# snap-research/F8Net

Measured on AMD Instinct MI355X. Metric: images/sec at bs=128 (ResNet-50 INT8), higher is better.
Workload: dtype int8 x int8 -> int32 (exact integer)

## Files before the change

### f8net_amd/csrc/f8_internal.h

```cpp
#pragma once
#include <hip/hip_runtime.h>
#include <stdint.h>
#include <stddef.h>

namespace f8 {

struct Options {
    int split = 2;
    int fuse_blocks = 1;
    int fuse_stages = -1;
    int fuse_dual = 1;
    int fuse_ds = 1;
    int fuse_opener = 1;
    int fuse_fc = 1;
    int fuse_stem = 1;
    int fuse_input = 1;
    int wstat = 1;
    int wstat_min_tiles = 2;
    int wstat_fast = 1;
    int s2wreg = 1;
    int wreg = 1;
    int fuse_bchain = 2;
    int fuse_bchain7 = 0;
    int fuse_chain = 1;
    int fuse_chain7 = 1;
    int fuse_pool = 1;
    int fuse_tail = 1;
    int chain_timeout_ms = 10000;
    int chain_stack = 1;
    int fuse_p12 = 1;
    int fuse_head2 = 1;
    int fuse_ir = 1;
    int fuse_irchain = 0;
    int fuse_dws = 0;
    int fuse_head_dws = 0;
    int fuse_dws7 = 0;
    int patch3x3 = 1;
    int dual_wide = 2048;
    int deep_nk = 7;
    int bk128 = 0;
    int dw_dot4 = 1;
    int dwk_dot4 = 1;
    int dw_mma = 1;
    int stem_rows = 1;
    int stem_grid_div = 0;
    int stem_wpc = 3;
    int opener_stg = 1;
    int chunk56 = -1, chunk28 = -1, chunk14 = -1;
    int chunk_budget_mb = 96;
    int chunk_ds = 1, chunk_opener = 0;
    int whole_batch_launches = 0;
    int pipeline_depth = 2;
    int shared_streams = 1;
    int arena_copies = 0;
    int split_streams = 1;
    int graph = 0;
    int stagger = -1, stagger_pipelined = 2;
    int check_device = 1;
    int requant_float = 0;
    int tap_tiled = 1;
    int check_input_range = 1;
};
void options_from_env(Options* o);
int* option_slot(Options* o, const char* key);

struct QuantOut {
    int8_t* ptr;
    int32_t n;
    int32_t lo, hi;
    uint32_t bias_xor;
// ... 274 lines not shown
inline bool dyn_lds_opted_in(unsigned long long* done, int* dev_out) {
    int dev = 0;
    if (hipGetDevice(&dev) != hipSuccess || dev < 0 || dev >= 64) { *dev_out = -1; return false; }
    *dev_out = dev;
    return ((*done >> dev) & 1ull) != 0;
}

struct ConvTile { int bm, bn, bk; };


bool pick_conv_tile(int M, int coutP, int ck, bool has_res, bool bk128, ConvTile* t);
int  conv_grid(const ConvTile& t, int M, int coutP);

int conv_inst(const ConvArgs& a, const ConvTile& t, bool res, bool dual, int deep_nk);
int conv_kernel_name(char* buf, size_t cap, const ConvArgs& a, const ConvTile& t, int inst);
hipError_t launch_conv(const ConvArgs& a, const ConvTile& t, int inst, hipStream_t s);
hipError_t launch_fused_bottleneck(const FusedArgs& a, hipStream_t s);
int fused_bottleneck_kernel_name(char* buf, size_t cap, const FusedArgs& a);
bool fused_bottleneck_supported(int C, int MID, int H, int W, int imgs_per_launch, int stage_mask, int* R);
bool fused_ds_supported(int C, int MID, int COUT, int H, int W, int* R);
bool fused_opener_supported(int C, int MID, int COUT, int H, int W, int* R);
int fused_opener_inst(const FusedArgs& a, bool stg);
int fused_opener_kernel_name(char* buf, size_t cap, const FusedArgs& a, int inst);
hipError_t launch_fused_opener(const FusedArgs& a, int inst, hipStream_t s);
bool chain_supported(int C, int MID, int H, int W, int cin0);
bool chain_tail_supported(int C, int MID, int H, int W, int cin0);
int chain_max_blocks(int C, int MID, int H, int W, int cin0, bool tail);
void chain_shape(int C, int MID, int H, int W, int cin0, bool tail, int* R, int* wg_per_cu);
bool chain_stackable(int C, int MID, int H, int W, int cin0, bool tail);
hipError_t launch_chain(const ChainArgs& a, int fast, int C, int MID, int H, int W, int cin0, hipStream_t s);
int chain_kernel_name(char* buf, size_t cap, int C, int MID, int H, int W, int cin0, bool tail, int fast);
bool cchain_supported(int C, int MID, int H, int W, int cin0, bool tail);
size_t cchain_xchg_bytes();
int cchain_clusters(int N, int slots);
int cchain_kernel_name(char* buf, size_t cap, int fast);
int chain_fast(const ChainArgs& a, unsigned shortcut_blocks, bool q8);
hipError_t launch_cchain(const ChainArgs& a, int fast, hipStream_t s);
bool bcchain_supported(int C, int H, int W, bool opener);
size_t bcchain_xchg_bytes();
int bcchain_inst(const BCChainArgs& a, bool q8);
int bcchain_kernel_name(char* buf, size_t cap, int inst);
hipError_t launch_bcchain(const BCChainArgs& a, int inst, hipStream_t s);
bool bchain_supported(int C, int H, int W);
bool bchain_ds_supported(int C, int H, int W);
int bchain_tiles_per_img(int C, int H, int W);
hipError_t launch_bchain(const BChainArgs& a, int fast, int C, int H, int W, hipStream_t s);
int bchain_fast(const BChainArgs& a, bool ds, bool q8);
// ... 79 lines not shown
```

### f8net_amd/csrc/f8_net.cpp

```cpp
#include "../../include/f8net.h"
#include "f8_internal.h"

#include <algorithm>
#include <cstdarg>
#include <cstdio>
#include <cstdlib>
#include <cstring>
#include <new>
#include <variant>
#include <string>
#include <mutex>
#include <vector>

using namespace f8;

namespace {

thread_local std::string g_err;

int fail(int code, const char* fmt, ...) {
    char buf[512];
    va_list ap;
    va_start(ap, fmt);
    vsnprintf(buf, sizeof buf, fmt, ap);
// ... 251 lines not shown
    {"fuse_tail", "F8_FUSE_TAIL", &Options::fuse_tail, 0, 1, true},
    {"fuse_chain7", "F8_FUSE_CHAIN7", &Options::fuse_chain7, 0, 1, true},
    {"fuse_pool", "F8_FUSE_POOL", &Options::fuse_pool, 0, 1, true},
    {"fuse_bchain", "F8_FUSE_BCHAIN", &Options::fuse_bchain, 0, 2, true},
    {"fuse_bchain7", "F8_FUSE_BCHAIN7", &Options::fuse_bchain7, 0, 2, true},
    {"chain_timeout_ms", "F8_CHAIN_TIMEOUT_MS", &Options::chain_timeout_ms, 0, 1 << 20, false},
    {"chain_stack", "F8_CHAIN_STACK", &Options::chain_stack, 0, 1, true},
    {"wreg", "F8_WREG", &Options::wreg, 0, 1, true},
    {"s2wreg", "F8_S2WREG", &Options::s2wreg, 0, 1, true},
    {"wstat", "F8_WSTAT", &Options::wstat, 0, 1, true},
    {"wstat_min_tiles", "F8_WSTAT_MIN_TILES", &Options::wstat_min_tiles, 0, 1 << 20, true},
    {"wstat_fast", "F8_WSTAT_FAST", &Options::wstat_fast, 0, 1, true},
    {"patch3x3", "F8_PATCH3X3", &Options::patch3x3, 0, 1, true},
    {"dual_wide", "F8_DUAL_WIDE", &Options::dual_wide, 0, 1 << 30, true},
    {"deep_nk", "F8_DEEP_NK", &Options::deep_nk, 1, 1 << 20, true},
    {"bk128", "F8_BK128", &Options::bk128, 0, 1, true},
    {"dw_dot4", "F8_DW_DOT4", &Options::dw_dot4, 0, 1, true},
    {"dw_mma", "F8_DW_MMA", &Options::dw_mma, 0, 1, true},
    {"dwk_dot4", "F8_DWK_DOT4", &Options::dwk_dot4, 0, 1, true},
    {"stem_wpc", "F8_STEM_WPC", &Options::stem_wpc, 1, 8, false},
    {"stem_rows", "F8_STEM_ROWS", &Options::stem_rows, 0, 1, true},
    {"stem_grid_div", "F8_STEM_GRID_DIV", &Options::stem_grid_div, 0, 32, false},
    {"opener_stg", "F8_OPENER_STG", &Options::opener_stg, 0, 1, true},
    {"chunk56", "F8_CHUNK", &Options::chunk56, -1, 1 << 20, false},
    {"chunk28", "F8_CHUNK28", &Options::chunk28, -1, 1 << 20, false},
    {"chunk14", "F8_CHUNK14", &Options::chunk14, -1, 1 << 20, false},
    {"chunk_budget_mb", "F8_CHUNK_BUDGET_MB", &Options::chunk_budget_mb, 1, 1 << 20, false},
    {"chunk_ds", "F8_CHUNK_DS", &Options::chunk_ds, 0, 1, false},
    {"chunk_opener", "F8_CHUNK_OPENER", &Options::chunk_opener, 0, 1, false},
    {"split_streams", "F8_SPLIT_STREAMS", &Options::split_streams, 0, 1, false},
    {"graph", "F8_GRAPH", &Options::graph, 0, 1, false},
    {"stagger", "F8_STAGGER", &Options::stagger, -1, 1 << 20, false},
    {"stagger_pipelined", "F8_STAGGER_PIPELINED", &Options::stagger_pipelined, 0, 1 << 20, false},
    {"check_device", "F8_CHECK_DEVICE", &Options::check_device, 0, 1, false},
    {"check_input_range", "F8_CHECK_INPUT_RANGE", &Options::check_input_range, 0, 1, false},
    {"requant_float", "F8_REQUANT_FLOAT", &Options::requant_float, 0, 1, true},
    {"pipeline_depth", "F8_PIPELINE_DEPTH", &Options::pipeline_depth, 2, 4, false},
    {"arena_copies", "F8_ARENA_COPIES", &Options::arena_copies, 0, 4, true},
    {"shared_streams", "F8_SHARED_STREAMS", &Options::shared_streams, 0, 1, true},
    {"whole_batch_launches", "F8_WHOLE_BATCH_LAUNCHES", &Options::whole_batch_launches, 0, 1, true},
    {"tap_tiled", "F8_TAP_TILED", &Options::tap_tiled, 0, 1, true},
};
static const OptKey* find_opt(const char* key) {
    if (!key) return nullptr;
    for (const auto& k : kOptKeys) if (!strcmp(k.key, key)) return &k;
    return nullptr;
// ... 2495 lines not shown
            a.x = (const int8_t*)fp(sF); a.x_bytes = (uint32_t)(sF.bytes_per_img * N); a.N = N;
            if (st.kind == S_STEMPOOL) a.wpc = net->opt.stem_wpc;
            a.grid_div = net->opt.stem_grid_div;
            if (st.raw_input && !(net->in_u8 && net->in_u8_nhwc)) {
                const size_t img = (size_t)sT.C * sT.H * sT.W;
                a.rC = sT.C; a.rH = sT.H; a.rW = sT.W; a.xor8 = sF.sgn ? 0u : 0x80808080u;
                if (net->in_u8) { a.raw_kind = 2; a.xu8 = net->in_u8 + (size_t)n0 * img; memcpy(a.lut, net->in_lut, sizeof a.lut); }
                else if (net->in_f32) { a.raw_kind = 1; a.xf = net->in_f32 + (size_t)n0 * img; a.scale = net->in_scale; a.qlo = net->in_lo; a.qhi = net->in_hi; }
                else {
                    a.raw_kind = 0; a.xi = input + (size_t)n0 * img;
                    if (net->opt.check_input_range) { a.err = net->d_err; a.chk_lo = sF.sgn ? -127 : 0; a.chk_hi = sF.sgn ? 127 : 255; }
                }
            }
            fill_out(&a.out32, a.q);
            e = launch_stem_pool(a, st.inst, s);
            break;
        }
        case S_FUSED: case S_P12: {
            const Form& xF = T[st.src_t].forms[st.src_f];
            FusedArgs a = std::get<FusedArgs>(st.args);
            a.x8 = (const int8_t*)fp(xF); a.x_bytes = (uint32_t)(xF.bytes_per_img * N); a.N = N;
            if (st.res_t >= 0) a.xr = (const int32_t*)fp(T[st.res_t].forms[st.res_f]);
            fill_out(&a.out32, a.q);
            e = st.variant == V_OPENER ? launch_fused_opener(a, st.inst, s) : st.variant == V_P12 ? launch_fused_p12(a, s) : launch_fused_bottleneck(a, s);
            break;
        }
        case S_CHAIN: {
            ChainArgs a = std::get<ChainArgs>(st.args);
            const Form& xF = T[st.src_t].forms[st.src_f];
            if (xF.kind == FORM_I8) a.x8in = (const int8_t*)fp(xF); else a.xr = (const int32_t*)fp(xF);
            if (a.tail) a.m2in = (const int8_t*)fp(T[st.src2_t].forms[st.src2_f]);
            a.N = N;
            if ((a.NG = chain_launch_groups(net, st, N, &a.stack)) < 1) return F8_ERR_STATE;
            fill_out(&a.out32, a.q);
            if (const int rc = chain_scratch(a.cs)) return rc;
            e = launch_chain(a, st.inst, st.C, st.MID, st.H, st.W, st.cin0, s);
            break;
        }
        case S_BCHAIN: if (st.cluster) {
            BCChainArgs a = std::get<BCChainArgs>(st.args);
            const Tensor& xs = T[st.src_t];
            if (st.res_t >= 0) { a.m0in = (const int8_t*)fp(xs.forms[st.src_f]); a.x8sc = (const int8_t*)fp(T[st.res_t].forms[st.res_f]); }
            else a.xr = (const int32_t*)fp(xs.forms[st.src_f]);
            a.N = N;
            { int32_t one = 1; if ((a.NG = chain_launch_groups(net, st, N, &one)) < 1) return F8_ERR_STATE; }
            fill_out(&a.out32, a.q);
            if (const int rc = chain_scratch(a.cs)) return rc;
// ... 518 lines not shown
```

### f8net_amd/csrc/f8_opener.hip

```cpp
#include "f8_device.h"
#include <cstdlib>
#include <cstdio>

namespace f8 {

template <int C, int MID, int W, int R, int COUT>
struct OpenerCfg {
    static constexpr int WO = W / 2;
    static constexpr int PR = 2 * R + 1;
    static constexpr int NE = WO + 1, NO = WO;
    static constexpr int PW = NE + NO;
    static constexpr int P1_PX = PR * W, NP1 = (P1_PX + 31) / 32;
    static constexpr int OUT_PX = R * WO, NPO = (OUT_PX + 31) / 32;
    static constexpr int PATCH_BYTES = (PR * PW * MID + 255) / 256 * 256;
    static constexpr int X1_BYTES = NP1 * 32 * 64, W0_BYTES = MID * 64, STAGE1 = X1_BYTES + W0_BYTES;
    static constexpr int MID2_BYTES = NPO * 32 * MID, XS_BYTES = NPO * 32 * C;
    static constexpr int W2B = MID * 64, NS2 = 5;
    static constexpr int REG_B = MID2_BYTES + XS_BYTES + NS2 * W2B;
    static constexpr int REG_A = 2 * STAGE1 > REG_B ? 2 * STAGE1 : REG_B;
    static constexpr int BIAS_INTS = 2 * MID + 2 * COUT;
    static constexpr int LDS_BYTES = PATCH_BYTES + REG_A + BIAS_INTS * 4;
    static constexpr int STAGE3 = 64 * MID + 64 * C;
    static constexpr int STG_BYTES = NPO * 32 * 128;
};

template <int C, int MID, int W, int R, int COUT, bool STG, bool P12 = false, int FQ = 0>
__global__ void __launch_bounds__(512) __attribute__((amdgpu_waves_per_eu(2, 2)))
fused_opener_kernel(const FusedArgs a) {
    using Cfg = OpenerCfg<C, MID, W, R, COUT>;
    constexpr int WO = Cfg::WO, PR = Cfg::PR, NE = Cfg::NE, PW = Cfg::PW;
    constexpr int P1_PX = Cfg::P1_PX, NP1 = Cfg::NP1, OUT_PX = Cfg::OUT_PX, NPO = Cfg::NPO;
    constexpr int CM = MID / 32, CMW = CM / 2, NP1W = (NP1 + 3) / 4;
    constexpr int NK1 = C / 64, NK2 = 9 * (MID / 64), NC3 = COUT / 64, KK3 = MID / 32, KKS = C / 32, CH = MID / 64;
    constexpr int X1_BYTES = Cfg::X1_BYTES, STAGE1 = Cfg::STAGE1, W2B = Cfg::W2B, NS2 = Cfg::NS2, STAGE3 = Cfg::STAGE3;
    static_assert(NPO == 4 && CM % 2 == 0 && NP1 % 4 == 0, "4 pixel-tile groups x 2 channel-tile groups");
    static_assert(MID % 64 == 0 && C % 64 == 0 && COUT % 128 == 0, "K steps of 64 bytes, chunk pairs");
    static_assert(Cfg::LDS_BYTES <= 160 * 1024, "LDS");
    static_assert(2 * STAGE3 <= Cfg::PATCH_BYTES && STAGE3 <= NS2 * W2B, "P3 ring: two stages over the patch, one over the W2 ring");
    static_assert(!STG || (Cfg::PATCH_BYTES - 2 * STAGE3 >= Cfg::STG_BYTES && NS2 * W2B - STAGE3 >= Cfg::STG_BYTES), "staging buffers");
    constexpr int XL1 = X1_BYTES / 16 / 512;
    constexpr int WL0 = (MID * 4 + 511) / 512;
    constexpr int WL4 = 64 * MID / 16 / 512, WLS = 64 * C / 16 / 512, XSL = NPO * 32 * C / 16 / 512;
    static_assert(X1_BYTES % 8192 == 0 && (MID * 4) % 512 == 0 && WL4 >= 1 && WLS >= 1, "every wave issues every DMA instruction (compile-time wait counts)");
    constexpr int L1 = XL1 + WL0, L3 = WL4 + WLS;

    if constexpr (FQ == 1) set_fp_round_nearest_even();
    extern __shared__ __attribute__((aligned(16))) char lds[];
    char* const patch = lds;
    char* const regA = lds + Cfg::PATCH_BYTES;
    char* const mid2 = regA;
    char* const xs = regA + Cfg::MID2_BYTES;
    char* const w2ring = xs + Cfg::XS_BYTES;
    int* const bias_lds = (int*)(regA + Cfg::REG_A);
    auto p3slot = [&](int s) -> char* { return s < 2 ? patch + s * STAGE3 : w2ring; };
    auto stgbuf = [&](int b) -> char* { return b == 0 ? patch + 2 * STAGE3 : w2ring + STAGE3; };

    using S64 = Swz<64>;
    using SM = Swz<MID>;
    using SC = Swz<C>;

    const int tid = threadIdx.x;
    const int lane = tid & 63;
    const int wave = __builtin_amdgcn_readfirstlane(tid >> 6) & 7;
    const int wa = wave >> 1, wb = wave & 1;
    const int l31 = lane & 31, lh = lane >> 5;

    int t;
    {
        const int nwg = gridDim.x, bid = blockIdx.x, xcd = bid & 7, qq = nwg >> 3, rr = nwg & 7;
        t = (xcd < rr ? xcd * (qq + 1) : rr * (qq + 1) + (xcd - rr) * qq) + (bid >> 3);
    }
    const int HO = a.H >> 1;
    const int n = t / a.tiles_per_img, ti = t - n * a.tiles_per_img;
    const int p0 = ti * R;
    const int gp1 = (n * a.H + 2 * p0 - 1) * W;
    const int m_tile = (n * HO + p0) * WO;

    const __amdgpu_buffer_rsrc_t rx = __builtin_amdgcn_make_buffer_rsrc((void*)a.x8, 0, a.x_bytes, 0x00020000);
    const __amdgpu_buffer_rsrc_t rw0 = __builtin_amdgcn_make_buffer_rsrc((void*)a.w0, 0, a.w0_bytes, 0x00020000);
    const __amdgpu_buffer_rsrc_t rw2 = __builtin_amdgcn_make_buffer_rsrc((void*)a.w2, 0, a.w2_bytes, 0x00020000);
    const __amdgpu_buffer_rsrc_t rw4 = __builtin_amdgcn_make_buffer_rsrc((void*)a.w4, 0, a.w4_bytes, 0x00020000);
    const __amdgpu_buffer_rsrc_t rwsc = __builtin_amdgcn_make_buffer_rsrc((void*)a.wsc, 0, a.wsc_bytes, 0x00020000);

#ifdef F8_TRACE
    unsigned long long tt[8]; tt[0] = __builtin_readcyclecounter();
#define F8_OT(i) tt[i] = __builtin_readcyclecounter()
#else
#define F8_OT(i)
#endif

    for (int i = tid; i < (P12 ? 2 * MID : Cfg::BIAS_INTS); i += 512) {
        int v;
        if (i < MID) v = a.b0[i];
        else if (i < 2 * MID) v = a.b2[i - MID];
        else if (i < 2 * MID + COUT) v = a.b4[i - 2 * MID];
        else v = a.bsc[i - 2 * MID - COUT];
        bias_lds[i] = v;
    }
    {
        const unsigned z = a.xor1;
        const v4i zv = {(int)z, (int)z, (int)z, (int)z};
        if (tid < PR * (MID / 16)) *(v4i*)(patch + (tid / (MID / 16)) * PW * MID + (tid % (MID / 16)) * 16) = zv;
        if (p0 == 0)
            for (int o = tid * 16; o < PW * MID; o += 512 * 16) *(v4i*)(patch + o) = zv;
    }

    unsigned xb1[XL1];
#pragma unroll
    for (int i = 0; i < XL1; ++i) {
        const int idx = tid + i * 512;
        const int row = idx >> 2, chunk = (idx & 3) ^ S64::f(row);
        const int pr = row / W;
        const bool ok = row < P1_PX && (2 * p0 - 1 + pr) >= 0;
        xb1[i] = ok ? (unsigned)((gp1 + row) * C + chunk * 16) : kOOB;
// ... 59 lines not shown
        char* base = p3slot(slot);
#pragma unroll
        for (int j = 0; j < WL4; ++j) {
            const unsigned woff = w4b[j] + (unsigned)(c * 64 * MID);
            __builtin_amdgcn_raw_ptr_buffer_load_lds(rw4, (__attribute__((address_space(3))) void*)(base + j * 8192 + wave * 1024), 16, woff, 0, 0, 0);
        }
#pragma unroll
        for (int j = 0; j < WLS; ++j) {
            const unsigned woff = wsb[j] + (unsigned)(c * 64 * C);
            __builtin_amdgcn_raw_ptr_buffer_load_lds(rwsc, (__attribute__((address_space(3))) void*)(base + 64 * MID + j * 8192 + wave * 1024), 16, woff, 0, 0, 0);
        }
    };

    unsigned cof[2];
#pragma unroll
    for (int kk = 0; kk < 2; ++kk) cof[kk] = (unsigned)(((kk * 2 + lh) ^ S64::f(l31)) << 4);

    {
        v16i acc[NP1W][CMW];
#pragma unroll
        for (int i = 0; i < CMW; ++i)
#pragma unroll
            for (int g = 0; g < 4; ++g) {
                v4i bv = {0, 0, 0, 0};
                if constexpr (FQ != 0) bv = *(const v4i*)(a.b0 + (wb * CMW + i) * 32 + 8 * g + 4 * lh);
#pragma unroll
                for (int j = 0; j < NP1W; ++j)
#pragma unroll
                    for (int e = 0; e < 4; ++e) acc[j][i][4 * g + e] = bv[e];
            }
        issue_p1(0, 0);
        static_for<NK1>([&](auto kc) {
            constexpr int KS = decltype(kc)::value;
            wait_vmcnt<0>();
            asm volatile("s_waitcnt lgkmcnt(0)" ::: "memory");
            __builtin_amdgcn_s_barrier();
            if constexpr (KS + 1 < NK1) issue_p1(KS + 1, (KS + 1) & 1);
            const char* base = regA + (KS & 1) * STAGE1;
#pragma unroll
            for (int kk = 0; kk < 2; ++kk) {
                v4i wf[CMW], xf[NP1W];
#pragma unroll
                for (int i = 0; i < CMW; ++i) wf[i] = *(const v4i*)(base + X1_BYTES + ((wb * CMW + i) * 32 + l31) * 64 + cof[kk]);
#pragma unroll
                for (int j = 0; j < NP1W; ++j) xf[j] = *(const v4i*)(base + ((wa + 4 * j) * 32 + l31) * 64 + cof[kk]);
#pragma unroll
                for (int j = 0; j < NP1W; ++j)
#pragma unroll
                    for (int i = 0; i < CMW; ++i) acc[j][i] = __builtin_amdgcn_mfma_i32_32x32x32_i8(wf[i], xf[j], acc[j][i], 0, 0, 0);
            }
        });
        asm volatile("s_waitcnt lgkmcnt(0)" ::: "memory");
        __builtin_amdgcn_s_barrier();
        F8_OT(1);
        if constexpr (!P12) issue_xs();
#pragma unroll
        for (int k = 0; k < NS2 - 1; ++k) issue_w2(k, k);

        const int floor0 = a.relu_a ? 0 : INT32_MIN;
        const float sc1 = FQ == 1 ? requant_u8_scale(a.n1) : 0.0f;
        (void)floor0; (void)sc1;
#pragma unroll
        for (int j = 0; j < NP1W; ++j) {
            const int pix = (wa + 4 * j) * 32 + l31;
            const int pr = pix / W, pc = pix - pr * W + 1;
            const bool ok = pix < P1_PX && (2 * p0 - 1 + pr) >= 0;
            const int ent = pr * PW + ((pc & 1) ? NE + (pc >> 1) : (pc >> 1));
#pragma unroll
            for (int i = 0; i < CMW; ++i) {
                const int ct = wb * CMW + i;
                unsigned d[4];
#pragma unroll
                for (int g = 0; g < 4; ++g) {
                    if constexpr (FQ != 0) {
                        d[g] = requant_u8x4_sel<FQ == 2 ? 2 : 1>(acc[j][i][4 * g], acc[j][i][4 * g + 1], acc[j][i][4 * g + 2], acc[j][i][4 * g + 3], a.n1, sc1) ^ 0x80808080u;
                    } else {
                        const v4i bv = *(const v4i*)(bias_lds + ct * 32 + 8 * g + 4 * lh);
                        int y[4];
#pragma unroll
                        for (int e = 0; e < 4; ++e) y[e] = requant1(max((int)((unsigned)acc[j][i][4 * g + e] + (unsigned)bv[e]), floor0), a.n1, a.lo1, a.hi1);
                        d[g] = pack4(y[0], y[1], y[2], y[3]) ^ a.xor1;
                    }
                }
                auto s0 = __builtin_amdgcn_permlane32_swap(d[0], d[2], false, false);
                auto s1 = __builtin_amdgcn_permlane32_swap(d[1], d[3], false, false);
                if (ok) {
                    v4i o = {(int)s0[0], (int)s0[1], (int)s1[0], (int)s1[1]};
                    *(v4i*)(patch + SM::off(ent, ct * 2 + lh)) = o;
                }
            }
        }
    }
    F8_OT(2);

    const int opix = wa * 32 + l31;
    const bool opix_ok = opix < OUT_PX;
    const int m = m_tile + opix;

    {
        v16i acc[CMW];
        const int oc = opix_ok ? opix : OUT_PX - 1;
        const int orow = oc / WO, ocol = oc - orow * WO;
        const int pe[3] = {2 * orow * PW + ocol, 2 * orow * PW + NE + ocol, 2 * orow * PW + ocol + 1};
#pragma unroll
        for (int i = 0; i < CMW; ++i)
// ... 7 lines not shown
            constexpr int J = decltype(jc)::value;
            constexpr int BEFORE = J == 0 ? NS2 - 1 : ((J - 1 + NS2 < NK2) ? J - 1 + NS2 : NK2);
            constexpr int AFTER = (J + NS2 < NK2) ? J + NS2 : NK2;
            wait_vmcnt<(BEFORE - 1 - J) * WL0>();
            asm volatile("s_waitcnt lgkmcnt(0)" ::: "memory");
            __builtin_amdgcn_s_barrier();
            static_for<AFTER - BEFORE>([&](auto ic) { constexpr int S = BEFORE + decltype(ic)::value; issue_w2(S, S % NS2); });
            constexpr int TAP = J / CH, TC = J % CH, TR = TAP / 3, TS = TAP % 3;
            const char* base = w2ring + (J % NS2) * W2B;
            const int ent = pe[TS] + TR * PW;
#pragma unroll
            for (int kk = 0; kk < 2; ++kk) {
                const v4i xf = *(const v4i*)(patch + SM::off(ent, TC * 4 + kk * 2 + lh));
#pragma unroll
                for (int i = 0; i < CMW; ++i) {
                    const v4i wf = *(const v4i*)(base + ((wb * CMW + i) * 32 + l31) * 64 + cof[kk]);
                    acc[i] = __builtin_amdgcn_mfma_i32_32x32x32_i8(wf, xf, acc[i], 0, 0, 0);
                }
            }
        });
        F8_OT(3);
        asm volatile("s_waitcnt lgkmcnt(0)" ::: "memory");
        __builtin_amdgcn_s_barrier();
        if constexpr (!P12) {
            issue_p3(0, 0);
            asm volatile("" ::: "memory");
            issue_p3(1, 1);
            asm volatile("" ::: "memory");
        }

        const int floor0 = a.relu_b ? 0 : INT32_MIN;
        const float sc2 = FQ == 1 ? requant_u8_scale(a.n2) : 0.0f;
        (void)floor0; (void)sc2;
#pragma unroll
        for (int i = 0; i < CMW; ++i) {
            const int ct = wb * CMW + i;
            unsigned d[4];
#pragma unroll
            for (int g = 0; g < 4; ++g) {
                if constexpr (FQ != 0) {
                    d[g] = requant_u8x4_sel<FQ == 2 ? 2 : 1>(acc[i][4 * g], acc[i][4 * g + 1], acc[i][4 * g + 2], acc[i][4 * g + 3], a.n2, sc2) ^ 0x80808080u;
                } else {
                    int y[4];
#pragma unroll
                    for (int e = 0; e < 4; ++e) y[e] = requant1(max(acc[i][4 * g + e], floor0), a.n2, a.lo2, a.hi2);
                    d[g] = pack4(y[0], y[1], y[2], y[3]) ^ a.xor2;
                }
            }
            auto s0 = __builtin_amdgcn_permlane32_swap(d[0], d[2], false, false);
            auto s1 = __builtin_amdgcn_permlane32_swap(d[1], d[3], false, false);
            v4i o = {(int)s0[0], (int)s0[1], (int)s1[0], (int)s1[1]};
            if constexpr (P12) { if (opix_ok) *(v4i*)(a.q[0].ptr + (size_t)m * MID + ct * 32 + lh * 16) = o; }
            else *(v4i*)(mid2 + SM::off(opix, ct * 2 + lh)) = o;
        }
    }
    F8_OT(4);

    if constexpr (!P12) {
        const int floor1 = a.relu1 ? 0 : -2147483647 ;
        const bool stage0 = STG && a.q[0].ptr != nullptr;
        const int n_direct = (a.out32 ? 4 : 0) + ((!STG && a.q[0].ptr) ? 1 : 0) + (a.q[1].ptr ? 1 : 0);
        auto stores_of = [&](int x) { return x < 0 ? 0 : n_direct + ((stage0 && x >= 2 && !(x & 1)) ? 2 : 0); };
        auto flush_pair = [&](int c0) {
            const char* buf = stgbuf((c0 >> 1) & 1);
#pragma unroll
            for (int rr = 0; rr < 2; ++rr) {
                const int tq = tid + rr * 512;
                const int row = tq >> 3, c16 = tq & 7;
                const bool live = row < OUT_PX;
                const int rw = live ? row : OUT_PX - 1;
                if (live || lane == 0) {
                    const v4i v = *(const v4i*)(buf + rw * 128 + ((c16 ^ (rw & 7)) << 4));
                    *(v4i*)(a.q[0].ptr + (size_t)(m_tile + rw) * COUT + c0 * 64 + c16 * 16) = v;
                }
            }
        };
        v4i xf[KK3], xsf[KKS];
        static_for<NC3>([&](auto cc) {
            constexpr int c = decltype(cc)::value;
            wait_vmcnt_dyn(stores_of(c - 2) + (c + 1 < NC3 ? L3 : 0) + stores_of(c - 1));
            asm volatile("s_waitcnt lgkmcnt(0)" ::: "memory");
// ... 58 lines not shown
                    *(v4i*)(stgbuf((c >> 1) & 1) + opix * 128 + ((c16 ^ (opix & 7)) << 4)) = o;
                } else if (opix_ok) {
                    *(v4i*)(a.q[k].ptr + (size_t)m * COUT + cot + 16 * lh) = o;
                }
            }
        });
        if (stage0) {
            asm volatile("s_waitcnt lgkmcnt(0)" ::: "memory");
            __builtin_amdgcn_s_barrier();
            flush_pair(NC3 - 2);
        }
    }
#ifdef F8_TRACE
    if (a.trace && tid == 0) {
        asm volatile("s_waitcnt vmcnt(0)" ::: "memory");
        tt[5] = __builtin_readcyclecounter();
        unsigned long long* tp = (unsigned long long*)a.trace + (size_t)blockIdx.x * 8;
        for (int i = 0; i < 6; ++i) tp[i] = tt[i];
    }
#endif
}

template <int C, int MID, int W, int R, int COUT, bool STG, bool P12 = false, int FQ = 0>
static hipError_t launch_opener_t(const FusedArgs& a, hipStream_t s) {
    using Cfg = OpenerCfg<C, MID, W, R, COUT>;
    static unsigned long long attr_done = 0; int attr_dev = -1;
    if (!dyn_lds_opted_in(&attr_done, &attr_dev)) {
        hipError_t e = hipFuncSetAttribute((const void*)fused_opener_kernel<C, MID, W, R, COUT, STG, P12, FQ>, hipFuncAttributeMaxDynamicSharedMemorySize, Cfg::LDS_BYTES);
        if (e != hipSuccess) return e;
        if (attr_dev >= 0) attr_done |= 1ull << attr_dev;
    }
    const int grid = a.N * a.tiles_per_img;
#ifdef F8_TRACE
    static unsigned long long* tbuf = nullptr; static int count = 0;
    static const int want = [] { const char* e = getenv("F8_TRACE_OPENER"); return e ? atoi(e) : -1; }();
    FusedArgs b = a;
    const bool tracing = (count++ == want);
    if (tracing) { if (!tbuf) (void)hipMalloc((void**)&tbuf, (size_t)1 << 22); (void)hipMemsetAsync(tbuf, 0, (size_t)grid * 64, s); b.trace = tbuf; }
    hipLaunchKernelGGL((fused_opener_kernel<C, MID, W, R, COUT, STG, P12, FQ>), dim3(grid), dim3(512), Cfg::LDS_BYTES, s, b);
    if (tracing) {
        (void)hipStreamSynchronize(s);
        unsigned long long* h = new unsigned long long[(size_t)grid * 8];
        (void)hipMemcpy(h, tbuf, (size_t)grid * 64, hipMemcpyDeviceToHost);
        double ph[5] = {0, 0, 0, 0, 0}; int n = 0;
        for (int i = 0; i < grid; ++i) { unsigned long long* p = h + (size_t)i * 8; if (!p[5]) continue; ++n; for (int k = 0; k < 5; ++k) ph[k] += (double)(p[k + 1] - p[k]); }
        fprintf(stderr, "[trace opener<%d,%d,%d,%d,%d>] grid %d: avg cycles per WG: P1 loop %.0f | P1 epi %.0f | P2 loop %.0f | P2 epi %.0f | P3 %.0f\n", C, MID, W, R, COUT, grid,
                ph[0] / n, ph[1] / n, ph[2] / n, ph[3] / n, ph[4] / n);
        delete[] h;
    }
    return hipGetLastError();
#else
    hipLaunchKernelGGL((fused_opener_kernel<C, MID, W, R, COUT, STG, P12, FQ>), dim3(grid), dim3(512), Cfg::LDS_BYTES, s, a);
    return hipGetLastError();
#endif
}

int fused_opener_inst(const FusedArgs& a, bool stg) {
    if (!a.p12only) return stg ? 1 : 0;
    const bool fqf = a.relu_a && a.relu_b && a.n1 > 0 && a.n2 > 0 && a.n1 <= 30 && a.n2 <= 30 && a.lo1 == 0 && a.lo2 == 0 && a.hi1 == 255 && a.hi2 == 255 &&
                     a.xor1 == 0x80808080u && a.xor2 == 0x80808080u;
#ifndef F8_OPENER_FQ
#define F8_OPENER_FQ 1
#endif
    return (!fqf || !F8_OPENER_FQ) ? 0 : ((a.rq_int || !a.acc_ok || a.n1 > kRequantU8MaxShift || a.n2 > kRequantU8MaxShift) ? 2 : 1);
}

int fused_opener_kernel_name(char* buf, size_t cap, const FusedArgs& a, int inst) {
    return snprintf(buf, cap, "f8::fused_opener_kernel<%d, %d, %d, %d, %d, %s, %s, %d>", a.C, a.MID, a.W, a.R, a.COUT, !a.p12only && inst ? "true" : "false",
                    a.p12only ? "true" : "false", a.p12only ? inst : 0);
}

hipError_t launch_fused_opener(const FusedArgs& a, int inst, hipStream_t s) {
    if (a.C == 256 && a.MID == 128 && a.COUT == 512 && a.W == 56 && a.R == 4) {
        if (a.p12only) {
            if (!(a.q[0].ptr && !a.q[1].ptr && !a.out32)) return hipErrorInvalidValue;
            const int fq = inst;
            return fq == 1 ? launch_opener_t<256, 128, 56, 4, 512, false, true, 1>(a, s) : fq == 2 ? launch_opener_t<256, 128, 56, 4, 512, false, true, 2>(a, s)
                                                                                               : launch_opener_t<256, 128, 56, 4, 512, false, true, 0>(a, s);
        }
        return inst ? launch_opener_t<256, 128, 56, 4, 512, true>(a, s) : launch_opener_t<256, 128, 56, 4, 512, false>(a, s);
    }
    return hipErrorInvalidValue;
}

bool fused_opener_supported(int C, int MID, int COUT, int H, int W, int* R) {
    if (C == 256 && MID == 128 && COUT == 512 && W == 56 && H % 8 == 0) { *R = 4; return true; }
    return false;
}

}
```

Baseline: 161,200.

## Make P12 opener kernel persistent with cross-tile prefetch of next tile's P1 stages

Splits the P12-only opener path into a dedicated persistent device routine. Each workgroup loops over a contiguous range of tiles (XCD-aware assignment), and the grid is capped at the CU count, optionally lower via a new F8_OPENER_WGS option. The first P1 stages of the next tile are issued during and after the current tile's P2, and biases are staged in LDS once per workgroup, so launch and pipeline fill costs are hidden. The trade-off is fewer workgroups, a tighter LDS ring layout with more complex vmcnt accounting, and possible load imbalance across tiles.

```diff
diff --git a/f8net_amd/csrc/f8_internal.h b/f8net_amd/csrc/f8_internal.h
--- a/f8net_amd/csrc/f8_internal.h
+++ b/f8net_amd/csrc/f8_internal.h
@@ -46,6 +46,7 @@
     int stem_grid_div = 0;
     int stem_wpc = 3;
     int opener_stg = 1;
+    int opener_wgs = 0;
     int chunk56 = -1, chunk28 = -1, chunk14 = -1;
     int chunk_budget_mb = 96;
     int chunk_ds = 1, chunk_opener = 0;
@@ -366,7 +367,7 @@
 bool fused_opener_supported(int C, int MID, int COUT, int H, int W, int* R);
 int fused_opener_inst(const FusedArgs& a, bool stg);
 int fused_opener_kernel_name(char* buf, size_t cap, const FusedArgs& a, int inst);
-hipError_t launch_fused_opener(const FusedArgs& a, int inst, hipStream_t s);
+hipError_t launch_fused_opener(const FusedArgs& a, int inst, int num_cu, int opener_wgs, hipStream_t s);
 bool chain_supported(int C, int MID, int H, int W, int cin0);
 bool chain_tail_supported(int C, int MID, int H, int W, int cin0);
 int chain_max_blocks(int C, int MID, int H, int W, int cin0, bool tail);
diff --git a/f8net_amd/csrc/f8_net.cpp b/f8net_amd/csrc/f8_net.cpp
--- a/f8net_amd/csrc/f8_net.cpp
+++ b/f8net_amd/csrc/f8_net.cpp
@@ -297,6 +297,7 @@
     {"stem_rows", "F8_STEM_ROWS", &Options::stem_rows, 0, 1, true},
     {"stem_grid_div", "F8_STEM_GRID_DIV", &Options::stem_grid_div, 0, 32, false},
     {"opener_stg", "F8_OPENER_STG", &Options::opener_stg, 0, 1, true},
+    {"opener_wgs", "F8_OPENER_WGS", &Options::opener_wgs, 0, 256, false},
     {"chunk56", "F8_CHUNK", &Options::chunk56, -1, 1 << 20, false},
     {"chunk28", "F8_CHUNK28", &Options::chunk28, -1, 1 << 20, false},
     {"chunk14", "F8_CHUNK14", &Options::chunk14, -1, 1 << 20, false},
@@ -2838,7 +2839,7 @@
             a.x8 = (const int8_t*)fp(xF); a.x_bytes = (uint32_t)(xF.bytes_per_img * N); a.N = N;
             if (st.res_t >= 0) a.xr = (const int32_t*)fp(T[st.res_t].forms[st.res_f]);
             fill_out(&a.out32, a.q);
-            e = st.variant == V_OPENER ? launch_fused_opener(a, st.inst, s) : st.variant == V_P12 ? launch_fused_p12(a, s) : launch_fused_bottleneck(a, s);
+            e = st.variant == V_OPENER ? launch_fused_opener(a, st.inst, net->num_cu, net->opt.opener_wgs, s) : st.variant == V_P12 ? launch_fused_p12(a, s) : launch_fused_bottleneck(a, s);
             break;
         }
         case S_CHAIN: {
diff --git a/f8net_amd/csrc/f8_opener.hip b/f8net_amd/csrc/f8_opener.hip
--- a/f8net_amd/csrc/f8_opener.hip
+++ b/f8net_amd/csrc/f8_opener.hip
@@ -24,6 +24,298 @@
     static constexpr int STG_BYTES = NPO * 32 * 128;
 };
 
+template <int C, int MID, int W, int R, int COUT, int FQ>
+__device__ __forceinline__ void opener_p12_tiles(const FusedArgs& a, char* const lds) {
+    using Cfg = OpenerCfg<C, MID, W, R, COUT>;
+    constexpr int WO = Cfg::WO, PR = Cfg::PR, NE = Cfg::NE, PW = Cfg::PW;
+    constexpr int P1_PX = Cfg::P1_PX, NP1 = Cfg::NP1, OUT_PX = Cfg::OUT_PX;
+    constexpr int CM = MID / 32, CMW = CM / 2, NP1W = (NP1 + 3) / 4;
+    constexpr int NK1 = C / 64, NK2 = 9 * (MID / 64), CH = MID / 64;
+    constexpr int X1_BYTES = Cfg::X1_BYTES, STAGE1 = Cfg::STAGE1, W2B = Cfg::W2B, NS2 = Cfg::NS2;
+    constexpr int XL1 = X1_BYTES / 16 / 512, WL0 = (MID * 4 + 511) / 512, L1 = XL1 + WL0;
+    constexpr int NST = CMW;
+    static_assert(STAGE1 <= Cfg::PATCH_BYTES && 2 * STAGE1 <= Cfg::REG_A, "P1 ring: slots 0 and 1 in REG_A, slot 2 over the patch");
+    static_assert(STAGE1 <= Cfg::MID2_BYTES + Cfg::XS_BYTES, "slot 0 (the next tile's stage 0, in flight during P2) lies below the W2 ring");
+    static_assert(NK1 >= 3 && NK2 > NS2 && OUT_PX > 3 * 32, "three stages up front; a prefetch step inside P2; no wave without a live output pixel");
+    static_assert(P1_PX > (XL1 - 1) * 128 && W <= 128, "dead gather rows: only in the last DMA instruction; image row -1: only in the first");
+
+    if constexpr (FQ == 1) set_fp_round_nearest_even();
+    char* const patch = lds;
+    char* const regA = lds + Cfg::PATCH_BYTES;
+    char* const w2ring = regA + Cfg::MID2_BYTES + Cfg::XS_BYTES;
+    int* const bias_lds = (int*)(regA + Cfg::REG_A);
+    auto p1slot = [&](int s) -> char* { return s == 2 ? patch : regA + s * STAGE1; };
+
+    using S64 = Swz<64>;
+    using SM = Swz<MID>;
+
+    const int tid = threadIdx.x;
+    const int wave = __builtin_amdgcn_readfirstlane(tid >> 6) & 7;
+    const int wa = wave >> 1, wb = wave & 1;
+#define F8_LANES                                                                                            \
+    int tq_ = tid; asm volatile("" : "+v"(tq_));                                                            \
+    const int lane = tq_ & 63, l31 = lane & 31, lh = lane >> 5;                                             \
+    unsigned cof[2];                                                                                        \
+    _Pragma("unroll") for (int kk = 0; kk < 2; ++kk) cof[kk] = (unsigned)(((kk * 2 + lh) ^ S64::f(l31)) << 4); \
+    (void)cof
+
+    int t, t_end, gx;
+    {
+        const int tiles = a.N * a.tiles_per_img, nwg = gridDim.x, bid = blockIdx.x;
+        const int nx = nwg < 8 ? nwg : 8, xcd = bid % nx, li = bid / nx, qq = tiles / nx, rr = tiles % nx;
+        gx = (nwg - xcd + nx - 1) / nx;
+        t = (xcd < rr ? xcd * (qq + 1) : rr * (qq + 1) + (xcd - rr) * qq);
+        t_end = t + qq + (xcd < rr ? 1 : 0);
+        t += li;
+    }
+    if (t >= t_end) return;
+
+    const __amdgpu_buffer_rsrc_t rx = __builtin_amdgcn_make_buffer_rsrc((void*)a.x8, 0, a.x_bytes, 0x00020000);
+    const __amdgpu_buffer_rsrc_t rw0 = __builtin_amdgcn_make_buffer_rsrc((void*)a.w0, 0, a.w0_bytes, 0x00020000);
+    const __amdgpu_buffer_rsrc_t rw2 = __builtin_amdgcn_make_buffer_rsrc((void*)a.w2, 0, a.w2_bytes, 0x00020000);
+
+#ifdef F8_TRACE
+    unsigned long long tt[5], tsum[4] = {0, 0, 0, 0}, tfirst = 0; int ntile = 0;
+#define F8_OT(i) tt[i] = __builtin_readcyclecounter()
+#else
+#define F8_OT(i)
+#endif
+
+    for (int i = tid; i < 2 * MID; i += 512) bias_lds[i] = i < MID ? a.b0[i] : a.b2[i - MID];
+
+    auto issue_p1 = [&](int ks, int gp, bool top) {
+        char* base = p1slot(ks % 3);
+        const unsigned tb = (unsigned)(gp * C + ks * 64);
+        int tq = tid; asm volatile("" : "+v"(tq));
+#pragma unroll
+        for (int i = 0; i < XL1; ++i) {
+            const int idx = tq + i * 512;
+            const int row = idx >> 2, chunk = (idx & 3) ^ S64::f(row);
+            const bool dead = (i == 0 && top && row < W) || (i == XL1 - 1 && row >= P1_PX);
+            const unsigned off = dead ? kOOB : (unsigned)(row * C + chunk * 16) + tb;
+            __builtin_amdgcn_raw_ptr_buffer_load_lds(rx, (__attribute__((address_space(3))) void*)(base + i * 8192 + wave * 1024), 16, off, 0, 0, 0);
+        }
+#pragma unroll
+        for (int j = 0; j < WL0; ++j) {
+            const int idx = tq + j * 512;
+            const int row = idx >> 2, chunk = (idx & 3) ^ S64::f(row);
+            const unsigned woff = (unsigned)(row * C + chunk * 16 + ks * 64);
+            __builtin_amdgcn_raw_ptr_buffer_load_lds(rw0, (__attribute__((address_space(3))) void*)(base + X1_BYTES + j * 8192 + wave * 1024), 16, woff, 0, 0, 0);
+        }
+    };
+    auto issue_w2 = [&](int j2, int slot, unsigned w2lane) {
+        char* base = w2ring + slot * W2B;
+#pragma unroll
+        for (int j = 0; j < WL0; ++j) {
+            const unsigned woff = w2lane + (unsigned)(j * 128 * 9 * MID + j2 * 64);
+            __builtin_amdgcn_raw_ptr_buffer_load_lds(rw2, (__attribute__((address_space(3))) void*)(base + j * 8192 + wave * 1024), 16, woff, 0, 0, 0);
+        }
+    };
+    auto w2_lane_offset = [&](int tq) { const int row = tq >> 2, chunk = (tq & 3) ^ S64::f(row); return (unsigned)(row * (9 * MID) + chunk * 16); };
+
+    const int HO = a.H >> 1;
+    __syncthreads();
+    {
+        const int n = t / a.tiles_per_img, p0 = (t - n * a.tiles_per_img) * R;
+        const int gp1 = (n * a.H + 2 * p0 - 1) * W;
+#pragma unroll
+        for (int k = 0; k < 3; ++k) { issue_p1(k, gp1, p0 == 0); asm volatile("" ::: "memory"); }
+    }
+    bool first = true;
+
+    do {
+        const int n = t / a.tiles_per_img, p0 = (t - n * a.tiles_per_img) * R;
+        const int gp1 = (n * a.H + 2 * p0 - 1) * W;
+        const int m_tile = (n * HO + p0) * WO;
+        const int tn = t + gx;
+        const bool has_next = tn < t_end;
+        const int nn = tn / a.tiles_per_img, p0n = (tn - nn * a.tiles_per_img) * R;
+        const int gp1n = (nn * a.H + 2 * p0n - 1) * W;
+        F8_OT(0);
+
+        {
+            v16i acc[NP1W][CMW];
+            {
+            F8_LANES;
+#pragma unroll
+            for (int i = 0; i < CMW; ++i)
+#pragma unroll
+                for (int g = 0; g < 4; ++g) {
+                    v4i bv = {0, 0, 0, 0};
+                    if constexpr (FQ != 0) bv = *(const v4i*)(bias_lds + (wb * CMW + i) * 32 + 8 * g + 4 * lh);
+#pragma unroll
+                    for (int j = 0; j < NP1W; ++j)
+#pragma unroll
+                        for (int e = 0; e < 4; ++e) acc[j][i][4 * g + e] = bv[e];
+                }
+            static_for<NK1>([&](auto kc) {
+                constexpr int KS = decltype(kc)::value;
+                constexpr int NEWER = ((KS + 1 > 2 ? KS + 1 : 2) < NK1 - 1 ? (KS + 1 > 2 ? KS + 1 : 2) : NK1 - 1) - KS;
+                if constexpr (KS == 0) { if (first) wait_vmcnt<NEWER * L1>(); else wait_vmcnt<NEWER * L1 + NST>(); }
+                else wait_vmcnt<NEWER * L1>();
+                asm volatile("s_waitcnt lgkmcnt(0)" ::: "memory");
+                __builtin_amdgcn_s_barrier();
+                if constexpr (KS >= 1 && KS + 2 < NK1) issue_p1(KS + 2, gp1, p0 == 0);
+                const char* base = p1slot(KS % 3);
+#pragma unroll
+                for (int kk = 0; kk < 2; ++kk) {
+                    v4i wf[CMW], xf[NP1W];
+#pragma unroll
+                    for (int i = 0; i < CMW; ++i) wf[i] = *(const v4i*)(base + X1_BYTES + ((wb * CMW + i) * 32 + l31) * 64 + cof[kk]);
+#pragma unroll
+                    for (int j = 0; j < NP1W; ++j) xf[j] = *(const v4i*)(base + ((wa + 4 * j) * 32 + l31) * 64 + cof[kk]);
+#pragma unroll
+                    for (int j = 0; j < NP1W; ++j)
+#pragma unroll
+                        for (int i = 0; i < CMW; ++i) acc[j][i] = __builtin_amdgcn_mfma_i32_32x32x32_i8(wf[i], xf[j], acc[j][i], 0, 0, 0);
+                }
+            });
+            }
+            asm volatile("s_waitcnt lgkmcnt(0)" ::: "memory");
+            __builtin_amdgcn_s_barrier();
+            F8_OT(1);
+            F8_LANES;
+            {
+                const unsigned w2lane = w2_lane_offset(tq_);
+#pragma unroll
+                for (int k = 0; k < NS2 - 1; ++k) issue_w2(k, k, w2lane);
+            }
+            {
+                const unsigned z = a.xor1;
+                const v4i zv = {(int)z, (int)z, (int)z, (int)z};
+                if (tq_ < PR * (MID / 16)) *(v4i*)(patch + (tq_ / (MID / 16)) * PW * MID + (tq_ % (MID / 16)) * 16) = zv;
+                if (p0 == 0)
+                    for (int o = tq_ * 16; o < PW * MID; o += 512 * 16) *(v4i*)(patch + o) = zv;
+            }
+
+            const int floor0 = a.relu_a ? 0 : INT32_MIN;
+            const float sc1 = FQ == 1 ? requant_u8_scale(a.n1) : 0.0f;
+            (void)floor0; (void)sc1;
+#pragma unroll
+            for (int j = 0; j < NP1W; ++j) {
+                const int pix = (wa + 4 * j) * 32 + l31;
+                const int pr = pix / W, pc = pix - pr * W + 1;
+                const bool ok = pix < P1_PX && (2 * p0 - 1 + pr) >= 0;
+                const int ent = pr * PW + ((pc & 1) ? NE + (pc >> 1) : (pc >> 1));
+#pragma unroll
+                for (int i = 0; i < CMW; ++i) {
+                    const int ct = wb * CMW + i;
+                    unsigned d[4];
+#pragma unroll
+                    for (int g = 0; g < 4; ++g) {
+                        if constexpr (FQ != 0) {
+                            d[g] = requant_u8x4_sel<FQ == 2 ? 2 : 1>(acc[j][i][4 * g], acc[j][i][4 * g + 1], acc[j][i][4 * g + 2], acc[j][i][4 * g + 3], a.n1, sc1) ^ 0x80808080u;
+                        } else {
+                            const v4i bv = *(const v4i*)(bias_lds + ct * 32 + 8 * g + 4 * lh);
+                            int y[4];
+#pragma unroll
+                            for (int e = 0; e < 4; ++e) y[e] = requant1(max((int)((unsigned)acc[j][i][4 * g + e] + (unsigned)bv[e]), floor0), a.n1, a.lo1, a.hi1);
+                            d[g] = pack4(y[0], y[1], y[2], y[3]) ^ a.xor1;
+                        }
+                    }
+                    auto s0 = __builtin_amdgcn_permlane32_swap(d[0], d[2], false, false);
+                    auto s1 = __builtin_amdgcn_permlane32_swap(d[1], d[3], false, false);
+                    if (ok) {
+                        v4i o = {(int)s0[0], (int)s0[1], (int)s1[0], (int)s1[1]};
+                        *(v4i*)(patch + SM::off(ent, ct * 2 + lh)) = o;
+                    }
+                }
+            }
+        }
+        F8_OT(2);
+
+        {
+            F8_LANES;
+            const unsigned w2lane = w2_lane_offset(tq_);
+            const int opix = wa * 32 + l31;
+            const bool opix_ok = opix < OUT_PX;
+            const int m = m_tile + opix;
+            v16i acc[CMW];
+            const int oc = opix_ok ? opix : OUT_PX - 1;
+            const int orow = oc / WO, ocol = oc - orow * WO;
+            const int pe[3] = {2 * orow * PW + ocol, 2 * orow * PW + NE + ocol, 2 * orow * PW + ocol + 1};
+#pragma unroll
+            for (int i = 0; i < CMW; ++i)
+#pragma unroll
+                for (int g = 0; g < 4; ++g) {
+                    const v4i bv = *(const v4i*)(bias_lds + MID + (wb * CMW + i) * 32 + 8 * g + 4 * lh);
+#pragma unroll
+                    for (int e = 0; e < 4; ++e) acc[i][4 * g + e] = bv[e];
+                }
+            static_for<NK2>([&](auto jc) {
+                constexpr int J = decltype(jc)::value;
+                constexpr int BEFORE = J == 0 ? NS2 - 1 : ((J - 1 + NS2 < NK2) ? J - 1 + NS2 : NK2);
+                constexpr int AFTER = (J + NS2 < NK2) ? J + NS2 : NK2;
+                constexpr bool PF = BEFORE < NK2 && AFTER == NK2;
+                if constexpr (BEFORE == NK2) { if (has_next) wait_vmcnt<(BEFORE - 1 - J) * WL0 + L1>(); else wait_vmcnt<(BEFORE - 1 - J) * WL0>(); }
+                else wait_vmcnt<(BEFORE - 1 - J) * WL0>();
+                asm volatile("s_waitcnt lgkmcnt(0)" ::: "memory");
+                __builtin_amdgcn_s_barrier();
+                static_for<AFTER - BEFORE>([&](auto ic) { constexpr int S = BEFORE + decltype(ic)::value; issue_w2(S, S % NS2, w2lane); });
+                if constexpr (PF) { if (has_next) { asm volatile("" ::: "memory"); issue_p1(0, gp1n, p0n == 0); } }
+                constexpr int TAP = J / CH, TC = J % CH, TR = TAP / 3, TS = TAP % 3;
+                const char* base = w2ring + (J % NS2) * W2B;
+                const int ent = pe[TS] + TR * PW;
+#pragma unroll
+                for (int kk = 0; kk < 2; ++kk) {
+                    const v4i xf = *(const v4i*)(patch + SM::off(ent, TC * 4 + kk * 2 + lh));
+#pragma unroll
+                    for (int i = 0; i < CMW; ++i) {
+                        const v4i wf = *(const v4i*)(base + ((wb * CMW + i) * 32 + l31) * 64 + cof[kk]);
+                        acc[i] = __builtin_amdgcn_mfma_i32_32x32x32_i8(wf, xf, acc[i], 0, 0, 0);
+                    }
+                }
+            });
+            F8_OT(3);
+            asm volatile("s_waitcnt lgkmcnt(0)" ::: "memory");
+            __builtin_amdgcn_s_barrier();
+
+            const int floor0 = a.relu_b ? 0 : INT32_MIN;
+            const float sc2 = FQ == 1 ? requant_u8_scale(a.n2) : 0.0f;
+            (void)floor0; (void)sc2;
+#pragma unroll
+            for (int i = 0; i < CMW; ++i) {
+                const int ct = wb * CMW + i;
+                unsigned d[4];
+#pragma unroll
+                for (int g = 0; g < 4; ++g) {
+                    if constexpr (FQ != 0) {
+                        d[g] = requant_u8x4_sel<FQ == 2 ? 2 : 1>(acc[i][4 * g], acc[i][4 * g + 1], acc[i][4 * g + 2], acc[i][4 * g + 3], a.n2, sc2) ^ 0x80808080u;
+                    } else {
+                        int y[4];
+#pragma unroll
+                        for (int e = 0; e < 4; ++e) y[e] = requant1(max(acc[i][4 * g + e], floor0), a.n2, a.lo2, a.hi2);
+                        d[g] = pack4(y[0], y[1], y[2], y[3]) ^ a.xor2;
+                    }
+                }
+                auto s0 = __builtin_amdgcn_permlane32_swap(d[0], d[2], false, false);
+                auto s1 = __builtin_amdgcn_permlane32_swap(d[1], d[3], false, false);
+                v4i o = {(int)s0[0], (int)s0[1], (int)s1[0], (int)s1[1]};
+                if (opix_ok) *(v4i*)(a.q[0].ptr + (size_t)m * MID + ct * 32 + lh * 16) = o;
+            }
+        }
+        asm volatile("" ::: "memory");
+        if (has_next) { issue_p1(1, gp1n, p0n == 0); asm volatile("" ::: "memory"); issue_p1(2, gp1n, p0n == 0); }
+        F8_OT(4);
+#ifdef F8_TRACE
+        for (int i = 0; i < 4; ++i) tsum[i] += tt[i + 1] - tt[i];
+        if (first) tfirst = tt[1] - tt[0];
+        ++ntile;
+#endif
+        first = false;
+        t = tn;
+    } while (t < t_end);
+#ifdef F8_TRACE
+    if (a.trace && tid == 0) {
+        unsigned long long* tp = (unsigned long long*)a.trace + (size_t)blockIdx.x * 8;
+        for (int i = 0; i < 4; ++i) tp[i] = tsum[i];
+        tp[4] = tfirst; tp[5] = (unsigned long long)ntile;
+    }
+#endif
+#undef F8_OT
+#undef F8_LANES
+}
+
 template <int C, int MID, int W, int R, int COUT, bool STG, bool P12 = false, int FQ = 0>
 __global__ void __launch_bounds__(512) __attribute__((amdgpu_waves_per_eu(2, 2)))
 fused_opener_kernel(const FusedArgs a) {
@@ -44,8 +336,9 @@
     static_assert(X1_BYTES % 8192 == 0 && (MID * 4) % 512 == 0 && WL4 >= 1 && WLS >= 1, "every wave issues every DMA instruction (compile-time wait counts)");
     constexpr int L1 = XL1 + WL0, L3 = WL4 + WLS;
 
-    if constexpr (FQ == 1) set_fp_round_nearest_even();
     extern __shared__ __attribute__((aligned(16))) char lds[];
+    if constexpr (P12) { opener_p12_tiles<C, MID, W, R, COUT, FQ>(a, lds); return; }
+    static_assert(P12 || FQ == 0, "FQ: P12 instances only");
     char* const patch = lds;
     char* const regA = lds + Cfg::PATCH_BYTES;
     char* const mid2 = regA;
@@ -89,7 +382,7 @@
 #define F8_OT(i)
 #endif
 
-    for (int i = tid; i < (P12 ? 2 * MID : Cfg::BIAS_INTS); i += 512) {
+    for (int i = tid; i < Cfg::BIAS_INTS; i += 512) {
         int v;
         if (i < MID) v = a.b0[i];
         else if (i < 2 * MID) v = a.b2[i - MID];
@@ -195,12 +488,10 @@
         for (int i = 0; i < CMW; ++i)
 #pragma unroll
             for (int g = 0; g < 4; ++g) {
-                v4i bv = {0, 0, 0, 0};
-                if constexpr (FQ != 0) bv = *(const v4i*)(a.b0 + (wb * CMW + i) * 32 + 8 * g + 4 * lh);
 #pragma unroll
                 for (int j = 0; j < NP1W; ++j)
 #pragma unroll
-                    for (int e = 0; e < 4; ++e) acc[j][i][4 * g + e] = bv[e];
+                    for (int e = 0; e < 4; ++e) acc[j][i][4 * g + e] = 0;
             }
         issue_p1(0, 0);
         static_for<NK1>([&](auto kc) {
@@ -226,13 +517,11 @@
         asm volatile("s_waitcnt lgkmcnt(0)" ::: "memory");
         __builtin_amdgcn_s_barrier();
         F8_OT(1);
-        if constexpr (!P12) issue_xs();
+        issue_xs();
 #pragma unroll
         for (int k = 0; k < NS2 - 1; ++k) issue_w2(k, k);
 
         const int floor0 = a.relu_a ? 0 : INT32_MIN;
-        const float sc1 = FQ == 1 ? requant_u8_scale(a.n1) : 0.0f;
-        (void)floor0; (void)sc1;
 #pragma unroll
         for (int j = 0; j < NP1W; ++j) {
             const int pix = (wa + 4 * j) * 32 + l31;
@@ -245,15 +534,11 @@
                 unsigned d[4];
 #pragma unroll
                 for (int g = 0; g < 4; ++g) {
-                    if constexpr (FQ != 0) {
-                        d[g] = requant_u8x4_sel<FQ == 2 ? 2 : 1>(acc[j][i][4 * g], acc[j][i][4 * g + 1], acc[j][i][4 * g + 2], acc[j][i][4 * g + 3], a.n1, sc1) ^ 0x80808080u;
-                    } else {
-                        const v4i bv = *(const v4i*)(bias_lds + ct * 32 + 8 * g + 4 * lh);
-                        int y[4];
-#pragma unroll
-                        for (int e = 0; e < 4; ++e) y[e] = requant1(max((int)((unsigned)acc[j][i][4 * g + e] + (unsigned)bv[e]), floor0), a.n1, a.lo1, a.hi1);
-                        d[g] = pack4(y[0], y[1], y[2], y[3]) ^ a.xor1;
-                    }
+                    const v4i bv = *(const v4i*)(bias_lds + ct * 32 + 8 * g + 4 * lh);
+                    int y[4];
+#pragma unroll
+                    for (int e = 0; e < 4; ++e) y[e] = requant1(max((int)((unsigned)acc[j][i][4 * g + e] + (unsigned)bv[e]), floor0), a.n1, a.lo1, a.hi1);
+                    d[g] = pack4(y[0], y[1], y[2], y[3]) ^ a.xor1;
                 }
                 auto s0 = __builtin_amdgcn_permlane32_swap(d[0], d[2], false, false);
                 auto s1 = __builtin_amdgcn_permlane32_swap(d[1], d[3], false, false);
@@ -307,41 +592,32 @@
         F8_OT(3);
         asm volatile("s_waitcnt lgkmcnt(0)" ::: "memory");
         __builtin_amdgcn_s_barrier();
-        if constexpr (!P12) {
-            issue_p3(0, 0);
-            asm volatile("" ::: "memory");
-            issue_p3(1, 1);
-            asm volatile("" ::: "memory");
-        }
+        issue_p3(0, 0);
+        asm volatile("" ::: "memory");
+        issue_p3(1, 1);
+        asm volatile("" ::: "memory");
 
         const int floor0 = a.relu_b ? 0 : INT32_MIN;
-        const float sc2 = FQ == 1 ? requant_u8_scale(a.n2) : 0.0f;
-        (void)floor0; (void)sc2;
 #pragma unroll
         for (int i = 0; i < CMW; ++i) {
             const int ct = wb * CMW + i;
             unsigned d[4];
 #pragma unroll
             for (int g = 0; g < 4; ++g) {
-                if constexpr (FQ != 0) {
-                    d[g] = requant_u8x4_sel<FQ == 2 ? 2 : 1>(acc[i][4 * g], acc[i][4 * g + 1], acc[i][4 * g + 2], acc[i][4 * g + 3], a.n2, sc2) ^ 0x80808080u;
-                } else {
-                    int y[4];
-#pragma unroll
-                    for (int e = 0; e < 4; ++e) y[e] = requant1(max(acc[i][4 * g + e], floor0), a.n2, a.lo2, a.hi2);
-                    d[g] = pack4(y[0], y[1], y[2], y[3]) ^ a.xor2;
-                }
+                int y[4];
+#pragma unroll
+                for (int e = 0; e < 4; ++e) y[e] = requant1(max(acc[i][4 * g + e], floor0), a.n2, a.lo2, a.hi2);
+                d[g] = pack4(y[0], y[1], y[2], y[3]) ^ a.xor2;
             }
             auto s0 = __builtin_amdgcn_permlane32_swap(d[0], d[2], false, false);
             auto s1 = __builtin_amdgcn_permlane32_swap(d[1], d[3], false, false);
             v4i o = {(int)s0[0], (int)s0[1], (int)s1[0], (int)s1[1]};
-            if constexpr (P12) { if (opix_ok) *(v4i*)(a.q[0].ptr + (size_t)m * MID + ct * 32 + lh * 16) = o; }
-            else *(v4i*)(mid2 + SM::off(opix, ct * 2 + lh)) = o;
+            *(v4i*)(mid2 + SM::off(opix, ct * 2 + lh)) = o;
         }
     }
     F8_OT(4);
 
-    if constexpr (!P12) {
+    {
         const int floor1 = a.relu1 ? 0 : -2147483647 ;
         const bool stage0 = STG && a.q[0].ptr != nullptr;
         const int n_direct = (a.out32 ? 4 : 0) + ((!STG && a.q[0].ptr) ? 1 : 0) + (a.q[1].ptr ? 1 : 0);
@@ -446,7 +722,7 @@
 }
 
 template <int C, int MID, int W, int R, int COUT, bool STG, bool P12 = false, int FQ = 0>
-static hipError_t launch_opener_t(const FusedArgs& a, hipStream_t s) {
+static hipError_t launch_opener_t(const FusedArgs& a, int num_cu, int wgs, hipStream_t s) {
     using Cfg = OpenerCfg<C, MID, W, R, COUT>;
     static unsigned long long attr_done = 0; int attr_dev = -1;
     if (!dyn_lds_opted_in(&attr_done, &attr_dev)) {
@@ -454,7 +730,12 @@
         if (e != hipSuccess) return e;
         if (attr_dev >= 0) attr_done |= 1ull << attr_dev;
     }
-    const int grid = a.N * a.tiles_per_img;
+    int grid = a.N * a.tiles_per_img;
+    if (P12) {
+        if (num_cu <= 0) num_cu = 256;
+        if (grid > num_cu) grid = num_cu;
+        if (wgs > 0 && grid > wgs) grid = wgs;
+    }
 #ifdef F8_TRACE
     static unsigned long long* tbuf = nullptr; static int count = 0;
     static const int want = [] { const char* e = getenv("F8_TRACE_OPENER"); return e ? atoi(e) : -1; }();
@@ -467,6 +748,14 @@
         unsigned long long* h = new unsigned long long[(size_t)grid * 8];
         (void)hipMemcpy(h, tbuf, (size_t)grid * 64, hipMemcpyDeviceToHost);
         double ph[5] = {0, 0, 0, 0, 0}; int n = 0;
+        if (P12) {
+            double f1 = 0; int nw = 0;
+            for (int i = 0; i < grid; ++i) { unsigned long long* p = h + (size_t)i * 8; if (!p[5]) continue; ++nw; n += (int)p[5]; f1 += (double)p[4]; for (int k = 0; k < 4; ++k) ph[k] += (double)p[k]; }
+            fprintf(stderr, "[trace opener<%d,%d,%d,%d,%d> P12] grid %d, %d tiles: avg cycles per tile: P1 loop %.0f | P1 epi %.0f | P2 loop %.0f | P2 epi + next issue %.0f || first tile of a WG: P1 loop %.0f | later tiles: P1 loop %.0f\n",
+                    C, MID, W, R, COUT, grid, n, ph[0] / n, ph[1] / n, ph[2] / n, ph[3] / n, f1 / nw, n > nw ? (ph[0] - f1) / (n - nw) : 0.0);
+            delete[] h;
+            return hipGetLastError();
+        }
         for (int i = 0; i < grid; ++i) { unsigned long long* p = h + (size_t)i * 8; if (!p[5]) continue; ++n; for (int k = 0; k < 5; ++k) ph[k] += (double)(p[k + 1] - p[k]); }
         fprintf(stderr, "[trace opener<%d,%d,%d,%d,%d>] grid %d: avg cycles per WG: P1 loop %.0f | P1 epi %.0f | P2 loop %.0f | P2 epi %.0f | P3 %.0f\n", C, MID, W, R, COUT, grid,
                 ph[0] / n, ph[1] / n, ph[2] / n, ph[3] / n, ph[4] / n);
@@ -494,15 +783,16 @@
                     a.p12only ? "true" : "false", a.p12only ? inst : 0);
 }
 
-hipError_t launch_fused_opener(const FusedArgs& a, int inst, hipStream_t s) {
+hipError_t launch_fused_opener(const FusedArgs& a, int inst, int num_cu, int wgs, hipStream_t s) {
     if (a.C == 256 && a.MID == 128 && a.COUT == 512 && a.W == 56 && a.R == 4) {
         if (a.p12only) {
             if (!(a.q[0].ptr && !a.q[1].ptr && !a.out32)) return hipErrorInvalidValue;
             const int fq = inst;
-            return fq == 1 ? launch_opener_t<256, 128, 56, 4, 512, false, true, 1>(a, s) : fq == 2 ? launch_opener_t<256, 128, 56, 4, 512, false, true, 2>(a, s)
-                                                                                               : launch_opener_t<256, 128, 56, 4, 512, false, true, 0>(a, s);
-        }
-        return inst ? launch_opener_t<256, 128, 56, 4, 512, true>(a, s) : launch_opener_t<256, 128, 56, 4, 512, false>(a, s);
+            return fq == 1 ? launch_opener_t<256, 128, 56, 4, 512, false, true, 1>(a, num_cu, wgs, s)
+                 : fq == 2 ? launch_opener_t<256, 128, 56, 4, 512, false, true, 2>(a, num_cu, wgs, s)
+                           : launch_opener_t<256, 128, 56, 4, 512, false, true, 0>(a, num_cu, wgs, s);
+        }
+        return inst ? launch_opener_t<256, 128, 56, 4, 512, true>(a, num_cu, wgs, s) : launch_opener_t<256, 128, 56, 4, 512, false>(a, num_cu, wgs, s);
     }
     return hipErrorInvalidValue;
 }
```

Result: no change. 162,500, median of 6 (+0.8%).
